# penumbra-zone/decaf377

Hardware: AMD Instinct MI355X
Metric: decaf377 var-base scalar-mults/sec + encodes/sec at 1/2/4/8 MI355X (higher is better)
Workload: dtype u32

## Files before the change

### decaf377_amd/csrc/curve.hpp

```cpp
#pragma once
#include "fq29.hpp"
#include "fqs29.hpp"

namespace d377 {

#include "constants.inc"

constexpr int GT_STRIDE = 12;
constexpr int S_HASH_BITS = 12;
struct SqrtTables {
  const uint32_t* gtab;
  const uint8_t* s_lookup;
  uint32_t* inv_fail;
};

#include "s_hash.inc"

D377_HD uint32_t s_hash_raw(const fe& x) {
  return ((x.l[0] ^ (x.l[1] << 3)) * D377_S_HASH_K) >> (32 - S_HASH_BITS);
}
D377_HD uint32_t s_hash(const fe& x) {
  D377_B(bound_require(x.vq < 1.0535, "s_lookup key must be below q + 2^248"));
  return s_hash_raw(x);
}
// ... 765 lines not shown
  F g = fe_sub(a, b);
  F f = fe_add(g, c);
  ge_of<F> r;
  r.x = fe_mul(e, f); r.y = fe_mul(g, h); r.z = fe_mul(f, g);
  r.t = p.t;
  if (with_t) r.t = fe_mul(e, h);
  return r;
}

D377_HD ge_of<fes> ge_double_neg_sq(const ge_of<fes>& p, bool with_t) {
  fes a = fe_sqr(p.x), b = fe_sqr(p.y);
  fes c = fe_sqr2x(p.z);
  fes s_ = fe_sqr(fe_sub(p.x, p.y));
  fes h = fe_add(a, b);
  fes e = fe_sub(h, s_);
  fes g = fe_sub(a, b);
  fes f = fe_add(g, c);
  ge_of<fes> r;
  r.x = fe_mul(e, f); r.y = fe_mul(g, h); r.z = fe_mul(f, g);
  r.t = p.t;
  if (with_t) r.t = fe_mul(e, h);
  return r;
}

D377_HD ge ge_double_latency(const ge& p) { return ge_double_fast(p, true); }

template <class F>
D377_HD gec_of<F> ge_to_cached(const ge_of<F>& p) {
  gec_of<F> c;
  if constexpr (std::is_same<F, fes>::value) c.ypx = fe_add(p.y, p.x);
  else c.ypx = fe_carry(fe_add(p.y, p.x));
  c.ymx = fe_sub(p.y, p.x);
  c.z2 = fe_dbl(p.z);
  c.kt = fe_mul(fe_as<F>(fe_const(FE_K)), p.t);
  return c;
}

template <class F>
D377_HD ge_of<F> ge_add_cached(const ge_of<F>& p, const gec_of<F>& q, bool neg, bool with_t) {
  F a = fe_mul(fe_sub_nc(p.y, p.x), q.ymx);
  F b = fe_mul(fe_add(p.y, p.x), q.ypx);
  F c = fe_mul(p.t, q.kt);
  F d = fe_mul(p.z, q.z2);
  F e = fe_sub(b, a), h = fe_add(b, a);
  F dmc = fe_sub(d, c), dpc = fe_add(d, c);
  F f = fe_select(neg, dpc, dmc), g = fe_select(neg, dmc, dpc);
  ge_of<F> r;
  r.x = fe_mul(e, f); r.y = fe_mul(g, h); r.z = fe_mul(f, g);
  r.t = p.t;
  if (with_t) r.t = fe_mul(e, h);
  return r;
}

struct gea { fe ypx, ymx, kt; };
D377_HD ge ge_add_affine(const ge& p, const gea& q, bool neg, bool with_t) {
  fe a = fe_mul(fe_sub_nc(p.y, p.x), q.ymx);
  fe b = fe_mul(fe_add(p.y, p.x), q.ypx);
  fe c = fe_mul(p.t, q.kt);
  fe d = fe_dbl(p.z);
  fe e = fe_sub(b, a), h = fe_add(b, a);
  fe dmc = fe_sub(d, c), dpc = fe_carry(fe_add(d, c));
  fe f = fe_select(neg, dpc, dmc), g = fe_select(neg, dmc, dpc);
  ge r;
  r.x = fe_mul(e, f); r.y = fe_mul(g, h); r.z = fe_mul(f, g);
  r.t = p.t;
  if (with_t) r.t = fe_mul(e, h);
  return r;
}

D377_HD gea gea_from_affine(const fe& x, const fe& y) {
  gea c;
  c.ypx = fe_carry(fe_add(y, x));
  c.ymx = fe_sub(y, x);
  c.kt = fe_mul(fe_mul(fe_const(FE_K), x), y);
  return c;
}
D377_HD ge ge_from_cached_affine(const gea& q, bool neg) {
  const fe one = fe_const(FE_ONE);
  ge r;
  r.x = fe_mul(fe_sub(q.ypx, fe_mul(q.ymx, one)), one);
  r.y = fe_mul(fe_add(q.ypx, q.ymx), one);
  r.z = fe_const(FE_TWO);
  const fe t = fe_mul(q.kt, fe_const(FE_2_OVER_K));
  r.t = fe_select(neg, fe_neg(t), t);
  return r;
}

template <class F>
D377_HD gec_of<F> gec_identity() {
  gec_of<F> id;
  id.ypx = fe_as<F>(fe_const(FE_ONE)); id.ymx = fe_as<F>(fe_const(FE_ONE)); id.z2 = fe_dbl(fe_as<F>(fe_const(FE_ONE)));
  id.kt = fe_as<F>(fe_zero());
  return id;
}
template <class Tab, class = void> struct tab_shares_identity { static constexpr bool value = false; };
template <class Tab> struct tab_shares_identity<Tab, std::void_t<decltype(Tab::shared_identity)>> { static constexpr bool value = Tab::shared_identity; };

template <class F = fe, class Tab>
D377_HD ge ge_scalar_mul_w4(const ge& p0, const uint32_t digits[8], Tab& tab, bool want_t = true) {
  const ge_of<F> p = ge_as<F>(p0);
  if constexpr (!tab_shares_identity<Tab>::value) tab.store(0, gec_identity<F>());
  const gec_of<F> pc = ge_to_cached(p);
  tab.store(1, pc);
  ge_of<F> acc = ge_double_fast(p, true);
  tab.store(2, ge_to_cached(acc));
#pragma unroll 1
  for (int j = 3; j <= 8; ++j) {
    acc = ge_add_cached(acc, pc, false, true);
    tab.store(j, ge_to_cached(acc));
  }
  int d = fr_digit(digits, 63);
  ge_of<F> r = ge_as<F>(ge_select(d != 0, p0, ge_identity()));
#pragma unroll 1
  for (int i = 62; i >= 0; --i) {
    d = fr_digit(digits, i);
    const bool neg = d < 0;
    const gec_of<F> e = tab.load(neg ? -d : d, neg);
#pragma unroll 1
    for (int j = 0; j < 4; ++j) r = ge_double_neg(r, j == 3);
    r = ge_add_cached(r, e, neg, want_t && i == 0);
  }
  return ge_unsigned(r);
}

template <class F = fes, class Tab>
D377_HD ge ge_scalar_mul_w4_lean(const ge& p0, const uint32_t digits[8], Tab& tab, bool want_t = true) {
  static_assert(std::is_same<F, fes>::value, "ge_double_neg_sq is priced and bounded for signed limbs");
  const ge_of<F> p = ge_as<F>(p0);
  if constexpr (!tab_shares_identity<Tab>::value) tab.store(0, gec_identity<F>());
  const gec_of<F> pc = ge_to_cached(p);
  tab.store(1, pc);
  ge_of<F> acc = ge_double_fast(p, true);
  tab.store(2, ge_to_cached(acc));
#pragma unroll 1
  for (int j = 3; j <= 8; ++j) {
    acc = ge_add_cached(acc, pc, false, true);
    tab.store(j, ge_to_cached(acc));
  }
  D377_B(bound_require(fr_digit(digits, 63) == 0 && fr_digit(digits, 62) >= 0 && fr_digit(digits, 62) <= 5,
                       "lean window chain: the scalar is not below r"));
  const int top = fr_digit(digits, 62) & 7;
  const gec_of<F> s = tab.load(top, false);
  ge_of<F> r;
  r.x = fe_carry(fe_sub(s.ypx, s.ymx)); r.y = fe_carry(fe_add(s.ypx, s.ymx)); r.z = fe_carry(s.z2);
  r.t = fe_as<F>(fe_zero());
#pragma unroll 1
  for (int i = 61; i >= 0; --i) {
    const int d = fr_digit(digits, i);
    const bool neg = d < 0;
    const gec_of<F> e = tab.load(neg ? -d : d, neg);
#pragma unroll 1
    for (int j = 0; j < 4; ++j) r = ge_double_neg_sq(r, j == 3);
    r = ge_add_cached(r, e, neg, want_t && i == 0);
  }
  return ge_unsigned(r);
}

D377_HD void fr_recode_signed256(const uint32_t k[8], int digits[32]) {
  uint32_t carry = 0;
#pragma unroll
  for (int i = 0; i < 32; ++i) {
    uint32_t d = ((k[i >> 2] >> (8 * (i & 3))) & 255u) + carry;
    carry = (d >= 128u) ? 1u : 0u;
    digits[i] = (int)d - (int)(carry << 8);
  }
}

#ifndef D377_FB_BITS
#define D377_FB_BITS 23
#endif
constexpr unsigned long long FB_R_TOP = 0x4aad95ull;
template <int BITS>
struct FbShape {
  static constexpr int bits = BITS;
  static constexpr int windows = (252 + BITS - 1) / BITS;
  static constexpr int entries = (1 << (BITS - 1)) + 1;
  static constexpr int top_bit = BITS * (windows - 1);
  static_assert(BITS >= 4 && BITS <= 23 && top_bit >= 228 && BITS * windows >= 252, "comb width");
  static_assert((FB_R_TOP >> (top_bit - 228)) + 1 < (1ull << (BITS - 1)), "the top digit of a scalar below r must not carry out");
  static_assert(windows >= 2, "the first window is peeled off the loop");
};
constexpr int FB_BITS = D377_FB_BITS;
constexpr int FB_WINDOWS = FbShape<FB_BITS>::windows;
constexpr int FB_ENTRIES = FbShape<FB_BITS>::entries;
template <int BITS = FB_BITS>
D377_HD int fb_digit(const uint32_t k[8], int i, uint32_t& carry) {
  const int bit = BITS * i, wi = bit >> 5, sh = bit & 31;
  uint32_t v = k[wi] >> sh;
  if (sh + BITS > 32 && wi + 1 < 8) v |= k[wi + 1] << (32 - sh);
  const uint32_t dd = (v & ((1u << BITS) - 1u)) + carry;
  carry = (dd >= (1u << (BITS - 1))) ? 1u : 0u;
  return (int)dd - (int)(carry << BITS);
}
template <int BITS = FB_BITS, class FTab>
D377_HD ge ge_scalar_mul_base_w8(const uint32_t k[8], const FTab& ftab, bool want_t = true) {
  constexpr int W = FbShape<BITS>::windows;
  uint32_t carry = 0;
  int d = fb_digit<BITS>(k, 0, carry);
  bool neg = d < 0;
  gea e = ftab.load(0, neg ? -d : d, neg);
  ge r;
  {
    const gea cur = e;
    const bool neg_cur = neg;
    d = fb_digit<BITS>(k, 1, carry);
    neg = d < 0;
    e = ftab.load(1, neg ? -d : d, neg);
    r = ge_from_cached_affine(cur, neg_cur);
  }
#pragma unroll 1
  for (int i = 1; i < W; ++i) {
    const gea cur = e;
    const bool neg_cur = neg;
    if (i + 1 < W) {
      d = fb_digit<BITS>(k, i + 1, carry);
      neg = d < 0;
      e = ftab.load(i + 1, neg ? -d : d, neg);
    }
    r = ge_add_affine(r, cur, neg_cur, want_t || i + 1 < W);
  }
  return r;
}
template <int BITS, class FTab, class KLoad>
D377_HD ge ge_fixed_msm_w8(int m, KLoad&& kload, const FTab& ftab, bool want_t = true) {
  constexpr int W = FbShape<BITS>::windows;
  uint32_t k[8];
  kload(0, k);
  uint32_t carry = 0;
  int d = fb_digit<BITS>(k, 0, carry);
  bool neg = d < 0;
  gea e = ftab.load(0, 0, neg ? -d : d, neg);
  ge r;
  {
    const gea cur = e;
    const bool neg_cur = neg;
    d = fb_digit<BITS>(k, 1, carry);
    neg = d < 0;
    e = ftab.load(0, 1, neg ? -d : d, neg);
    r = ge_from_cached_affine(cur, neg_cur);
  }
  const int total = m * W;
  int j = 0, i = 1;
#pragma unroll 1
  for (int s = 1; s < total; ++s) {
    const gea cur = e;
    const bool neg_cur = neg;
    if (s + 1 < total) {
      if (++i == W) {
        i = 0;
        ++j;
        kload(j, k);
        carry = 0;
      }
      d = fb_digit<BITS>(k, i, carry);
      neg = d < 0;
      e = ftab.load(j, i, neg ? -d : d, neg);
    }
    r = ge_add_affine(r, cur, neg_cur, want_t || s + 1 < total);
  }
  return r;
}
template <class FTab>
struct FbIndexedTabs {
  const FTab& tabs;
  int comb;
  D377_HD gea load(int, int i, int c, bool swap) const { return tabs.load(comb, i, c, swap); }
};
template <int BITS, class FTab, class TLoad>
D377_HD ge ge_fixed_msm_indexed_w8(int t, TLoad&& tload, const FTab& ftab, bool want_t = true) {
  FbIndexedTabs<FTab> it{ftab, 0};
  return ge_fixed_msm_w8<BITS>(t, [&](int j, uint32_t k[8]) { it.comb = tload(j, k); }, it, want_t);
}

D377_HD fe fe_pow_words(const fe& x, const uint32_t (&e)[8]) {
  fe r = fe_const(FE_ONE);
#pragma unroll 1
  for (int i = 255; i >= 0; --i) {
    r = fe_sqr(r);
    if ((e[i >> 5] >> (i & 31)) & 1u) r = fe_mul(r, x);
  }
  return r;
}
D377_HD fe fe_invert_pow(const fe& x) {
  const uint32_t ee[8] = {0xFFFFFFFFu, FQ_MODULUS_W_LIT[1] - 1u, FQ_MODULUS_W_LIT[2], FQ_MODULUS_W_LIT[3],
                          FQ_MODULUS_W_LIT[4], FQ_MODULUS_W_LIT[5], FQ_MODULUS_W_LIT[6], FQ_MODULUS_W_LIT[7]};
  return fe_pow_words(x, ee);
}

template <class PT>
D377_HD fe fe_invert_chain(const fe& x, PT& pt) {
  return fe_mul(fe_sqr_n(fe_pow_m12(x, pt), 48), fe_pow_2_47_m1(x));
}

D377_HD void fr_half_words(uint32_t k[8]) {
  const uint32_t odd = k[0] & 1u;
  uint64_t c = 0;
#pragma unroll
  for (int i = 0; i < 8; ++i) { c += (uint64_t)k[i] + (odd ? FR_ORDER_W_LIT[i] : 0u); k[i] = (uint32_t)c; c >>= 32; }
#pragma unroll
  for (int i = 0; i < 8; ++i) k[i] = (k[i] >> 1) | (i < 7 ? (k[i + 1] << 31) : 0u);
}

#ifndef D377_DCB_K
#define D377_DCB_K 8
#endif
constexpr int DCB_K = D377_DCB_K;
// ... 153 lines not shown
```

### decaf377_amd/csrc/d377.hip

```cpp
#include <hip/hip_runtime.h>
#include <stdint.h>
#include <stdio.h>
#include <stdlib.h>
#include <string.h>
#include <chrono>
#include <mutex>
#include <new>
#include <thread>
#include <type_traits>
#include <vector>

#include "../../include/decaf377_amd.h"
#include "curve.hpp"
#include "device_util.hpp"
#include "dcb.hpp"
#include "quad_ops.hpp"
#include "row_ops.hpp"
#include "host_state.hpp"
#include "codec_chunked.hpp"
#include "fixed_comb.hpp"

using namespace d377;

thread_local char d377_g_err[512] = "";

namespace {

template <class F>
struct GlobalTab {
  static_assert(std::is_same<F, fes>::value, "the packed slots hold signed-limb elements");
  static constexpr bool shared_identity = true;
  uint32_t* base;
  const uint32_t* ident;
  size_t nthreads, tid;
  __device__ __forceinline__ void store(int j, const gec_of<F>& c) {
    uint32_t* p = base + ((size_t)j * nthreads + tid) * VB_ENTRY_WORDS;
    slot_pack_store(p, c.ypx); slot_pack_store(p + PACKED_SLOT, c.ymx);
    slot_pack_store(p + 2 * PACKED_SLOT, c.z2); slot_pack_store(p + 3 * PACKED_SLOT, c.kt);
  }
  __device__ __forceinline__ gec_of<F> load(int j, bool swap) const {
    const uint32_t* own = base + ((size_t)j * nthreads + tid) * VB_ENTRY_WORDS;
    const uint32_t* p = j == 0 ? ident : own;
    gec_of<F> c;
    c.ypx = slot_unpack_load<F>(p + (swap ? PACKED_SLOT : 0));
    c.ymx = slot_unpack_load<F>(p + (swap ? 0 : PACKED_SLOT));
    c.z2 = slot_unpack_load<F>(p + 2 * PACKED_SLOT);
    c.kt = slot_unpack_load<F>(p + 3 * PACKED_SLOT);
    return c;
  }
};
template <int BITS>
struct FixedTab {
  const uint32_t* base;
  __device__ __forceinline__ gea load(int i, int j, bool swap) const {
    return pt_load_affine(base + ((size_t)i * FbShape<BITS>::entries + j) * FBW_ENTRY_WORDS, swap);
  }
};

__device__ fe fe_pow_u32(const fe& x, uint32_t e) {
  int top = 31 - __clz((int)e);
  fe r = x;
#pragma unroll 1
  for (int i = top - 1; i >= 0; --i) {
    r = fe_sqr(r);
    if ((e >> i) & 1u) r = fe_mul(r, x);
  }
  return r;
}

__global__ void __launch_bounds__(BLOCK) k_init_gtab(uint32_t* gtab) {
  const int idx = blockIdx.x * BLOCK + threadIdx.x;
  if (idx >= 6 * 256) return;
  const int t = idx >> 8, nu = idx & 255;
  fe base = fe_sqr_n(fe_const(FE_SQRT_G), 8 * t);
  fe v = nu == 0 ? fe_const(FE_ONE) : fe_pow_u32(base, (uint32_t)nu);
  v = fe_mul_strict(v, fe_const(FE_ONE));
  uint32_t* p = gtab + (size_t)idx * GT_STRIDE;
#pragma unroll
  for (int i = 0; i < NL; ++i) p[i] = v.l[i];
  p[9] = 0; p[10] = 0; p[11] = 0;
}

__global__ void k_init_vb_identity(uint32_t* rec) {
  if (blockIdx.x != 0 || threadIdx.x != 0) return;
  const gec_of<fes> id = gec_identity<fes>();
  slot_pack_store(rec, id.ypx); slot_pack_store(rec + PACKED_SLOT, id.ymx);
  slot_pack_store(rec + 2 * PACKED_SLOT, id.z2); slot_pack_store(rec + 3 * PACKED_SLOT, id.kt);
}

__global__ void __launch_bounds__(BLOCK) k_init_slookup(uint8_t* s_lookup, uint32_t* keys ,
                                                        int* collisions) {
  const int nu = threadIdx.x;
  fe b39 = fe_sqr_n(fe_const(FE_SQRT_G_INV), 39);
  fe v = nu == 0 ? fe_const(FE_ONE) : fe_pow_u32(b39, (uint32_t)nu);
  fe c = fe_reduce_once(fe_mul_strict(v, fe_const(FE_ONE)));
  keys[2 * nu] = s_hash_raw(c);
  uint32_t h2 = 0xFFFFFFFFu;
  if (c.l[NL - 1] < (1u << 16)) {
    fe cq = fe_add(c, fe_const(Q_LIMBS));
    uint32_t carry = 0;
    fe n;
#pragma unroll
    for (int i = 0; i < NL; ++i) {
      uint32_t t = cq.l[i] + carry;
      if (i < NL - 1) { n.l[i] = t & MASK29; carry = t >> RB; } else n.l[i] = t;
    }
    h2 = s_hash_raw(n);
  }
  keys[2 * nu + 1] = h2;
  for (int i = threadIdx.x; i < (1 << S_HASH_BITS); i += BLOCK) s_lookup[i] = 0;
  __syncthreads();
  if (threadIdx.x == 0) {
    int coll = 0;
    for (int k = 0; k < 256; ++k)
      for (int r = 0; r < 2; ++r) {
        uint32_t h = keys[2 * k + r];
        if (h == 0xFFFFFFFFu) continue;
        for (int k2 = 0; k2 < k; ++k2)
          for (int r2 = 0; r2 < 2; ++r2)
            if (keys[2 * k2 + r2] == h) ++coll;
        s_lookup[h] = (uint8_t)k;
      }
    *collisions = coll;
  }
}

template <int FB_BITS>
__global__ void k_init_fbase_bases(uint32_t* bases) {
  constexpr int FB_WINDOWS = FbShape<FB_BITS>::windows;
  if (blockIdx.x != 0 || threadIdx.x != 0) return;
  ge p = ge_generator();
#pragma unroll 1
  for (int i = 0; i < FB_WINDOWS; ++i) {
    slot_store(bases + (size_t)i * 4 * SLOT, p.x); slot_store(bases + (size_t)i * 4 * SLOT + SLOT, p.y);
    slot_store(bases + (size_t)i * 4 * SLOT + 2 * SLOT, p.z); slot_store(bases + (size_t)i * 4 * SLOT + 3 * SLOT, p.t);
#pragma unroll 1
    for (int k = 0; k < FB_BITS; ++k) p = ge_double(p);
  }
}
__global__ void __launch_bounds__(BLOCK, WAVES_PER_SIMD) k_sqrt_ratio_zeta(SqrtTables T, const uint8_t* num32,
                                                           const uint8_t* den32, size_t n,
                                                           uint8_t* root32, uint8_t* was_square, int min_curve_root, DcbScratch dcb) {
  D377_POW_LDS();
  D377_DCB_BEGIN(root32);
  dcb_rounds<1, false>(n, io, pt,
    [&](size_t i, int j) {
      uint32_t wd[8];
      load32(den32, i, wd);
      dcb_put_den(io, 0, j, fe_from_words_mod_order_strict(wd));
    },
    [&](size_t i, int j, const uint32_t (*invw)[8], bool have) {
      uint32_t wn[8], wd[8], wr[8];
      load32(num32, i, wn);
      load32(den32, i, wd);
      fe inv = fe_from_words(invw[0]);
      fe r;
      const bool ws = fe_sqrt_ratio_zeta<false>(T, pt, fe_from_words_mod_order_strict(wn), fe_from_words_mod_order_strict(wd), &r,
                                                min_curve_root != 0, &inv, have);
      fe_to_bytes_words(r, wr);
      store32(root32, i, wr);
      was_square[i] = ws ? 1 : 0;
    });
  D377_DCB_END();
}

constexpr int CODEC_CHUNKED_MIN = 2;
__global__ void __launch_bounds__(BLOCK, WAVES_PER_SIMD) k_decompress(SqrtTables T, const uint8_t* enc32, size_t n,
                                                      uint64_t* xyzt, uint8_t* status) {
  D377_POW_LDS();
  for (size_t i = (size_t)blockIdx.x * BLOCK + threadIdx.x; i < n; i += (size_t)gridDim.x * BLOCK) {
    uint32_t w[8];
    load32(enc32, i, w);
    ge g;
    const uint32_t bad = ge_decompress(T, pt, w, &g);
    status[i] = (uint8_t)bad;
    if (bad) {
      uint8_t* b = reinterpret_cast<uint8_t*>(xyzt);
      store32_zero(b, 4 * i); store32_zero(b, 4 * i + 1); store32_zero(b, 4 * i + 2); store32_zero(b, 4 * i + 3);
    } else {
      store_ge_mont256(xyzt, i, g);
    }
  }
}

__global__ void __launch_bounds__(BLOCK, WAVES_PER_SIMD) k_decompress_chunked(SqrtTables T, const uint8_t* enc32, size_t n,
                                                              uint64_t* xyzt, uint8_t* status, DcbScratch dcb) {
  D377_POW_LDS();
  D377_DCB_BEGIN(xyzt);
  dcb_rounds<1, false, false>(n, io, pt,
    [&](size_t i, int j) {
      uint32_t w[8];
      load32(enc32, i, w);
      dcb_put_den(io, 0, j, ge_decompress_den(w));
    },
    [&](size_t i, int, const uint32_t (*invw)[8], bool) {
      uint32_t w[8];
      load32(enc32, i, w);
      const fe inv = fe_from_words(invw[0]);
      ge g;
      const uint32_t bad = ge_decompress(T, pt, w, &g, &inv);
      status[i] = (uint8_t)bad;
      if (bad) {
        uint8_t* b = reinterpret_cast<uint8_t*>(xyzt);
        store32_zero(b, 4 * i); store32_zero(b, 4 * i + 1); store32_zero(b, 4 * i + 2); store32_zero(b, 4 * i + 3);
      } else {
        store_ge_mont256(xyzt, i, g);
      }
    });
  D377_DCB_END();
}

__global__ void __launch_bounds__(BLOCK, WAVES_PER_SIMD) k_compress(SqrtTables T, const uint64_t* xyzt, size_t n,
                                                    uint8_t* enc32) {
  D377_POW_LDS();
  for (size_t i = (size_t)blockIdx.x * BLOCK + threadIdx.x; i < n; i += (size_t)gridDim.x * BLOCK) {
    uint32_t w[8];
    ge_compress(T, pt, load_ge_mont256(xyzt, i), w);
    store32(enc32, i, w);
  }
}

__global__ void __launch_bounds__(BLOCK, WAVES_PER_SIMD) k_roundtrip(SqrtTables T, const uint8_t* enc32, size_t n,
                                                     uint8_t* out32, uint8_t* status) {
  D377_POW_LDS();
  for (size_t i = (size_t)blockIdx.x * BLOCK + threadIdx.x; i < n; i += (size_t)gridDim.x * BLOCK) {
    uint32_t w[8];
    load32(enc32, i, w);
    ge g;
    const uint32_t bad = ge_decompress(T, pt, w, &g);
    ge_compress(T, pt, g, w, bad == 0);
    status[i] = (uint8_t)bad;
    if (bad) store32_zero(out32, i); else store32(out32, i, w);
  }
}

__global__ void __launch_bounds__(BLOCK, WAVES_PER_SIMD) k_encode_to_curve(SqrtTables T, const uint8_t* fq32, size_t n,
                                                           uint8_t* out32, DcbScratch dcb) {
  D377_POW_LDS();
  D377_DCB_BEGIN(out32);
  dcb_rounds<1, true>(n, io, pt,
    [&](size_t i, int j) {
      uint32_t w[8];
      load32(fq32, i, w);
      dcb_put_den(io, 0, j, ge_elligator_den(fe_from_words_mod_order(w)));
    },
    [&](size_t i, int j, const uint32_t (*invw)[8], bool have) {
      uint32_t w[8];
      load32(fq32, i, w);
      fe inv = fe_from_words(invw[0]);
      fe s, t;
      ge_elligator_st(T, pt, fe_from_words_mod_order(w), &s, &t, &inv, have);
      D377_INVARIANT(T, ge_from_jacobi_st(s, t), true);
      dcb_put(io, j, ge_dcb_from_jacobi_st(s, t));
    });
  D377_DCB_END();
}

struct Words8 { uint32_t w[8]; };
template <class PT>
__device__ __forceinline__ Words8 hash_exceptional_words(SqrtTables T, PT pt, Words8 a1, Words8 a2) {
  fe s1, t1, s2, t2, unused = fe_zero();
  ge_elligator_st(T, pt, fe_from_words_mod_order(a1.w), &s1, &t1, &unused, false);
  ge_elligator_st(T, pt, fe_from_words_mod_order(a2.w), &s2, &t2, &unused, false);
  Words8 r;
  ge_compress(T, pt, ge_add(ge_from_jacobi_st(s1, t1), ge_from_jacobi_st(s2, t2)), r.w);
  return r;
}
template <class PT>
__device__ __forceinline__ void hash_exceptional_pair(SqrtTables T, PT pt, const uint8_t* r1, const uint8_t* r2, size_t i, uint32_t w[8]) {
  Words8 a1, a2;
  load32(r1, i, a1.w);
  load32(r2, i, a2.w);
  const Words8 r = hash_exceptional_words(T, pt, a1, a2);
#pragma unroll
  for (int k = 0; k < 8; ++k) w[k] = r.w[k];
}
__global__ void __launch_bounds__(BLOCK, WAVES_PER_SIMD) k_hash_to_curve(SqrtTables T, const uint8_t* r1, const uint8_t* r2,
                                                         size_t n, uint8_t* out32, DcbScratch dcb) {
  D377_POW_LDS();
  D377_DCB_BEGIN(out32);
  uint32_t flagged = 0;
  dcb_rounds<2, true>(n, io, pt,
    [&](size_t i, int j) {
      uint32_t w[8];
      load32(r1, i, w);
      dcb_put_den(io, 0, j, ge_elligator_den(fe_from_words_mod_order(w)));
      load32(r2, i, w);
      dcb_put_den(io, 1, j, ge_elligator_den(fe_from_words_mod_order(w)));
    },
    [&](size_t i, int j, const uint32_t (*invw)[8], bool have) {
      uint32_t w[8];
      load32(r1, i, w);
      fe inv = fe_from_words(invw[0]);
      fe s1, t1, s2, t2;
      ge_elligator_st(T, pt, fe_from_words_mod_order(w), &s1, &t1, &inv, have);
      load32(r2, i, w);
      inv = fe_from_words(invw[1]);
      ge_elligator_st(T, pt, fe_from_words_mod_order(w), &s2, &t2, &inv, have);
      D377_INVARIANT(T, ge_from_jacobi_st(s1, t1), true);
      D377_INVARIANT(T, ge_from_jacobi_st(s2, t2), true);
      bool exceptional;
      dcb_state st = ge_dcb_from_jacobi_sum(s1, t1, s2, t2, &exceptional);
#if defined(D377_CHECK_INVARIANTS)
      exceptional |= (i & 3) == 3;
#endif
      const dcb_state ne = dcb_neutral();
      st.p = fe_select(exceptional, ne.p, st.p); st.w = fe_select(exceptional, ne.w, st.w);
      st.n0 = fe_select(exceptional, ne.n0, st.n0); st.n1 = fe_select(exceptional, ne.n1, st.n1);
      dcb_put(io, j, st);
      if (exceptional) {
        flagged |= 1u << j;
        load32(r1, i, w);
        io.put(2, j, w);
        load32(r2, i, w);
        io.put(3, j, w);
      }
    },
    [&](DcbIO& io2, int cnt) {
      if (__any(flagged != 0)) {
#pragma unroll 1
        for (int j = 0; j < cnt; ++j) {
          const bool mine = ((flagged >> j) & 1u) != 0;
          if (!__any(mine)) continue;
          Words8 a1, a2;
          io2.get(2, j, a1.w);
          io2.get(3, j, a2.w);
          const Words8 r = hash_exceptional_words(T, pt, a1, a2);
          if (mine) io2.emit(j, r.w);
        }
      }
      flagged = 0;
    });
  D377_DCB_END();
}

__global__ void __launch_bounds__(BLOCK, WAVES_PER_SIMD) k_scalar_mul_var(SqrtTables T, const uint8_t* enc32,
                                                          const uint8_t* scalar32, size_t n, uint8_t* out32,
                                                          uint8_t* status, uint32_t* scratch, const uint32_t* vb_identity,
                                                          DcbScratch dcb) {
  D377_POW_LDS();
  D377_DCB_BEGIN(out32);
  GlobalTab<fes> tab;
  tab.base = scratch;
  tab.ident = vb_identity;
  tab.nthreads = (size_t)dcb.nslots * BLOCK;
  tab.tid = io.lane;
  dcb_rounds<1, true, false>(n, io, pt,
    [&](size_t i, int j) {
      uint32_t w[8];
      load32(enc32, i, w);
      dcb_put_den(io, 0, j, ge_decompress_den(w));
    },
    [&](size_t i, int j, const uint32_t (*invw)[8], bool have) {
      uint32_t w[8], k[8], dg[8];
      load32(enc32, i, w);
      load32(scalar32, i, k);
      const fe inv = fe_from_words(invw[0]);
      ge g;
      const uint32_t bad = ge_decompress<fes>(T, pt, w, &g, &inv);
      status[i] = (uint8_t)bad;
      fr_reduce_words(k);
      fr_half_words(k);
      fr_recode_signed16(k, dg);
      const ge r = ge_scalar_mul_w4_lean<fes>(g, dg, tab, DCB_WANT_T);
      D377_INVARIANT(T, r, bad == 0);
      dcb_put(io, j, ge_dcb_from_half(r, bad != 0));
    });
  D377_DCB_END();
}

template <int BITS>
__global__ void __launch_bounds__(BLOCK, FB_SETS) k_scalar_mul_base(SqrtTables T, const uint32_t* fbase,
                                                           const uint8_t* scalar32, size_t n, uint8_t* out32, DcbScratch dcb) {
  D377_POW_LDS();
  D377_DCB_BEGIN(out32);
  FixedTab<BITS> ft{fbase};
  dcb_rounds<0, true>(n, io, pt,
    [&](size_t, int) {},
    [&](size_t i, int j, const uint32_t (*)[8], bool) {
      uint32_t k[8];
      load32(scalar32, i, k);
      fr_reduce_words(k);
      fr_half_words(k);
      const ge r = ge_scalar_mul_base_w8<BITS>(k, ft, DCB_WANT_T);
      D377_INVARIANT(T, r, true);
      dcb_put(io, j, ge_dcb_from_half(r, false));
    });
  D377_DCB_END();
}

constexpr int SMALL_THREADS = 64;
constexpr int SMALL_QUADS = SMALL_THREADS / 4;
static_assert(GQ_TAB_ENTRIES == VB_ENTRIES, "the quad chain's table is the per-lane chain's: 0 .. 8 times P");
struct OneDcbIO {
  uint32_t st[4][8], parked_[8], out[8];
  __device__ __forceinline__ void put(int s, int, const uint32_t* w) { for (int k = 0; k < 8; ++k) st[s][k] = w[k]; }
  __device__ __forceinline__ void get(int s, int, uint32_t* w) const { for (int k = 0; k < 8; ++k) w[k] = st[s][k]; }
  __device__ __forceinline__ void park(int, const uint32_t* w) { for (int k = 0; k < 8; ++k) parked_[k] = w[k]; }
  __device__ __forceinline__ void parked(int, uint32_t* w) const { for (int k = 0; k < 8; ++k) w[k] = parked_[k]; }
  __device__ __forceinline__ void emit(int, const uint32_t* w) { for (int k = 0; k < 8; ++k) out[k] = w[k]; }
};
__device__ __forceinline__ fe fe_shfl_xor(const fe& a, int mask) {
  fe r;
#pragma unroll
  for (int i = 0; i < NL; ++i) r.l[i] = (uint32_t)__shfl_xor((int)a.l[i], mask);
  return r;
}
__device__ __forceinline__ fe quads16_invert(const fe& p) {
  const fe q0 = fe_shfl_xor(p, 4), p1 = fe_mul_strict(p, q0);
  const fe q1 = fe_shfl_xor(p1, 8), p2 = fe_mul_strict(p1, q1);
  const fe q2 = fe_shfl_xor(p2, 16), p3 = fe_mul_strict(p2, q2);
  const fe q3 = fe_shfl_xor(p3, 32);
  const fe inv = row::fe_invert_wave(fe_mul_strict(p3, q3));
  return fe_mul(fe_mul(fe_mul(fe_mul(inv, q3), q2), q1), q0);
}

template <bool ELEMENT>
__global__ void __launch_bounds__(SMALL_THREADS)
k_scalar_mul_var_small(SqrtTables T, const uint8_t* enc32, const uint8_t* scalar32, size_t n, uint8_t* out32, uint8_t* status) {
  __shared__ uint32_t lds_pow_[POW_TAB * NL * SMALL_THREADS];
  __shared__ uint32_t tab[SMALL_QUADS * VB_ENTRIES * GQ_WORDS];
  struct Pow64 {
    uint32_t* col;
    __device__ __forceinline__ void put(int j, const fe& v) { for (int k = 0; k < NL; ++k) col[(j * NL + k) * SMALL_THREADS] = v.l[k]; }
    __device__ __forceinline__ fe get(int j) const { fe r; for (int k = 0; k < NL; ++k) r.l[k] = col[(j * NL + k) * SMALL_THREADS]; return r; }
  } pt;
  pt.col = lds_pow_ + threadIdx.x;
  const int role = threadIdx.x & 3, quad = threadIdx.x >> 2;
  uint32_t* qtab = tab + quad * VB_ENTRIES * GQ_WORDS;
  for (size_t base = (size_t)blockIdx.x * SMALL_QUADS; base < n; base += (size_t)gridDim.x * SMALL_QUADS) {
    const bool active = base + quad < n;
    const size_t e = active ? base + quad : n - 1;
    uint32_t w[8], k[8], dg[8];
    load32(scalar32, e, k);
    ge g;
    uint32_t bad = 0;
    fr_reduce_words(k);
    if (ELEMENT) {
      g = load_ge_mont256(reinterpret_cast<const uint64_t*>(enc32), e);
    } else {
      load32(enc32, e, w);
      bad = ge_decompress(T, pt, w, &g);
      fr_half_words(k);
    }
    fr_recode_signed16(k, dg);
    const fe v = gq_scalar_mul_w4(gq_from_ge(g, role), dg, qtab, role);
    const ge r = gq_to_ge(v);
    D377_INVARIANT(T, r, bad == 0);
    if (ELEMENT) {
      if (active && role == 0) store_ge_mont256(reinterpret_cast<uint64_t*>(out32), e, r);
    } else {
      const dcb_state st = ge_dcb_from_half(r, bad != 0);
      uint32_t wo[8];
      dcb_encode_one(st, quads16_invert(st.p), wo);
      if (active && role == 0) {
        store32(out32, e, wo);
        status[e] = (uint8_t)bad;
      }
    }
    __syncthreads();
  }
}

template <int FB_BITS>
__device__ __forceinline__ fe fb_fetch_slot(const uint32_t* fbase, int role, int i, int d) {
  const int slot = gq_add_slot(role, d < 0);
  const uint32_t* src = fbase + ((size_t)i * FbShape<FB_BITS>::entries + (size_t)(d < 0 ? -d : d)) * FBW_ENTRY_WORDS + NL * (slot == 0 ? 1 : (slot == 1 ? 0 : 2));
  fe x = fe_const(FE_ONE);
  if (slot < 3) {
#pragma unroll
    for (int j = 0; j < NL; ++j) x.l[j] = src[j];
  }
  return x;
}
template <bool ELEMENT, int FB_BITS>
__global__ void __launch_bounds__(SMALL_THREADS)
k_scalar_mul_base_small(const uint32_t* fbase, const uint8_t* scalar32, size_t n, uint8_t* out) {
  constexpr int FB_WINDOWS = FbShape<FB_BITS>::windows;
  const int role = threadIdx.x & 3, quad = threadIdx.x >> 2;
  const size_t e_raw = (size_t)blockIdx.x * SMALL_QUADS + quad;
  const bool active = e_raw < n;
  const size_t e = active ? e_raw : n - 1;
  uint32_t k[8];
  load32(scalar32, e, k);
  fr_reduce_words(k);
  if (!ELEMENT) fr_half_words(k);
  uint32_t carry = 0;
  int d = fb_digit<FB_BITS>(k, 0, carry);
  fe nxt = fb_fetch_slot<FB_BITS>(fbase, role, 0, d);
  fe v = gq_from_ge(ge_identity(), role);
#pragma unroll 1
  for (int i = 0; i < FB_WINDOWS; ++i) {
    const fe cur = nxt;
    const bool neg = d < 0;
    if (i + 1 < FB_WINDOWS) {
      d = fb_digit<FB_BITS>(k, i + 1, carry);
      nxt = fb_fetch_slot<FB_BITS>(fbase, role, i + 1, d);
    }
    v = gq_add_with(v, cur, role, neg);
  }
  const ge r = gq_to_ge(v);
  if (ELEMENT) {
    if (active && role == 0) store_ge_mont256(reinterpret_cast<uint64_t*>(out), e, r);
  } else {
    const dcb_state st = ge_dcb_from_half(r, false);
    uint32_t w[8];
    dcb_encode_one(st, quads16_invert(st.p), w);
    if (active && role == 0) store32(out, e, w);
  }
}

template <bool ELEMENT>
__global__ void __launch_bounds__(64)
k_scalar_mul_var_tiny(SqrtTables T, const uint8_t* enc32, const uint8_t* scalar32, size_t n, uint8_t* out32, uint8_t* status) {
  __shared__ uint32_t tab[row::RQ_TAB_ENTRIES * row::RQ_WORDS];
  __shared__ uint32_t xrec[2 * row::RQ_WORDS];
  const int t = threadIdx.x;
// ... 1873 lines not shown
```

### decaf377_amd/csrc/fqs29.hpp

```cpp
#pragma once
#include <type_traits>
#include "fq29.hpp"

namespace d377 {

struct fes {
  int32_t l[NL];
#if defined(D377_BOUNDS)
  int64_t lo[NL], hi[NL];
  double vlo, vhi;
#endif
};

constexpr uint32_t Q2L[NL] = {0x00000002u, 0x01180000u, 0x00000085u, 0x09dbfb40u, 0x16002b35u,
                              0x0d1e5c37u, 0x0ab305a2u, 0x17a68b29u, 0x002556cau};

#if defined(D377_BOUNDS)
inline void sbound_limbs_int32(const fes& a, int64_t lim, const char* what) {
  for (int i = 0; i < NL; ++i) bound_require(a.lo[i] >= -lim && a.hi[i] < lim, what);
}
inline void sbound_product(const fes& a, const fes& b, bool square, int scale) {
  sbound_limbs_int32(a, (int64_t)1 << 31, "signed product: operand limb outside int32");
  sbound_limbs_int32(b, (int64_t)1 << 31, "signed product: operand limb outside int32");
  if (square) sbound_limbs_int32(a, (int64_t)1 << 30, "signed square: doubled limb outside int32");
  const __int128 lim = (__int128)1 << 63;
  __int128 clo = 0, chi = 0;
  for (int k = 0; k < 2 * NL - 1; ++k) {
    __int128 lo = clo, hi = chi;
    __int128 slo = clo, shi = chi;
    for (int i = 0; i < NL; ++i) {
      const int j = k - i;
      if (j < 0 || j >= NL) continue;
      const __int128 c[4] = {(__int128)a.lo[i] * b.lo[j], (__int128)a.lo[i] * b.hi[j],
                             (__int128)a.hi[i] * b.lo[j], (__int128)a.hi[i] * b.hi[j]};
      __int128 pmin = c[0], pmax = c[0];
      for (int t = 1; t < 4; ++t) { if (c[t] < pmin) pmin = c[t]; if (c[t] > pmax) pmax = c[t]; }
      pmin *= scale; pmax *= scale;
      slo += pmin; shi += pmax;
      if (pmin < 0) lo += pmin;
      if (pmax > 0) hi += pmax;
      if (j >= 1 && i < NL) {
        const __int128 red = -(__int128)MASK29 * QL[j];
        slo += red; lo += red;
      }
    }
    bound_require(lo >= -lim && hi < lim, "signed product column leaves +-2^63");
    clo = slo >= 0 ? slo >> RB : -((-slo + MASK29) >> RB);
    chi = shi >= 0 ? shi >> RB : -((-shi + MASK29) >> RB);
  }
}
inline void sbound_set_product(fes& r, const fes& a, const fes& b, double scale) {
  for (int i = 0; i < NL - 1; ++i) { r.lo[i] = 0; r.hi[i] = MASK29; }
  const double p[4] = {a.vlo * b.vlo, a.vlo * b.vhi, a.vhi * b.vlo, a.vhi * b.vhi};
  double pmin = p[0], pmax = p[0];
  for (int t = 1; t < 4; ++t) { if (p[t] < pmin) pmin = p[t]; if (p[t] > pmax) pmax = p[t]; }
  r.vlo = scale * pmin / R_OVER_Q - 1.0 - 1e-6;
  r.vhi = scale * pmax / R_OVER_Q + 1e-6;
  r.lo[NL - 1] = (int64_t)__builtin_floor(r.vlo * Q_TOP) - 1;
  r.hi[NL - 1] = (int64_t)__builtin_floor(r.vhi * Q_TOP) + 1;
  bound_require(r.lo[NL - 1] >= -((int64_t)1 << 31) && r.hi[NL - 1] < ((int64_t)1 << 31), "signed product: top limb outside int32");
}
inline void sbound_linear(fes& r, const char* what) { sbound_limbs_int32(r, (int64_t)1 << 31, what); }
#endif

template <bool SCALE2, bool SQUARE>
D377_HD fes fes_mul_ref(const fes& a, const fes& b) {
  uint64_t acc = 0;
  int32_t m[NL], a2[NL], b2[NL];
  fes r;
#pragma unroll
  for (int i = 0; i < NL; ++i) { a2[i] = (int32_t)((uint32_t)a.l[i] << 1); b2[i] = SCALE2 ? a2[i] : a.l[i]; }
#pragma unroll
  for (int k = 0; k < 2 * NL - 1; ++k) {
    const int lo = k < NL ? 0 : k - (NL - 1), hi = k < NL ? k : NL - 1;
    if (SQUARE) {
#pragma unroll
      for (int i = lo; 2 * i < k; ++i) acc += (uint64_t)((int64_t)a2[i] * b2[k - i]);
      if ((k & 1) == 0) acc += (uint64_t)((int64_t)b2[k / 2] * a.l[k / 2]);
    } else {
#pragma unroll
      for (int i = lo; i <= hi; ++i) acc += (uint64_t)((int64_t)a.l[i] * b.l[k - i]);
    }
#pragma unroll
    for (int i = lo; i < (k < NL ? k : NL); ++i) acc -= (uint64_t)((int64_t)m[i] * (int64_t)QL[k - i]);
    if (k < NL) m[k] = (int32_t)((uint32_t)acc & MASK29);
    else r.l[k - NL] = (int32_t)((uint32_t)acc & MASK29);
    acc = (uint64_t)((int64_t)acc >> RB);
  }
  r.l[NL - 1] = (int32_t)(uint32_t)acc;
  return r;
}

#if defined(__HIP_DEVICE_COMPILE__)
#define D377_ASM_NQ                                                                                     \
  "s"(-(int32_t)QL[1]), "s"(-(int32_t)QL[2]), "s"(-(int32_t)QL[3]), "s"(-(int32_t)QL[4]), "s"(-(int32_t)QL[5]), \
  "s"(-(int32_t)QL[6]), "s"(-(int32_t)QL[7]), "s"(-(int32_t)QL[8])
#endif

D377_HD fes fe_mul(const fes& a, const fes& b) {
  D377_B(sbound_product(a, b, false, 1); ++op_counts().mul);
#if defined(__HIP_DEVICE_COMPILE__)
  fes r; int64_t top; int32_t m8;
  asm(D377_ASM_SMUL : D377_ASM_OUT(r, top, m8) : D377_ASM_IN(a), D377_ASM_IN(b), D377_ASM_NQ : D377_ASM_CLOBBER);
  r.l[NL - 1] = (int32_t)top;
#else
  fes r = fes_mul_ref<false, false>(a, b);
#endif
  D377_B(sbound_set_product(r, a, b, 1.0));
  return r;
}
D377_HD fes fe_sqr(const fes& a) {
  D377_B(sbound_product(a, a, true, 1); ++op_counts().sqr);
#if defined(__HIP_DEVICE_COMPILE__)
  fes r; int64_t top; int32_t m8, t[8];
  asm(D377_ASM_SSQR : D377_ASM_OUT(r, top, m8), D377_ASM_TMP8(t) : D377_ASM_IN(a), D377_ASM_NQ : D377_ASM_CLOBBER);
  r.l[NL - 1] = (int32_t)top;
#else
  fes r = fes_mul_ref<false, true>(a, a);
#endif
  D377_B(sbound_set_product(r, a, a, 1.0));
  return r;
}
D377_HD fes fe_sqr2x(const fes& a) {
  D377_B(sbound_product(a, a, true, 2); ++op_counts().sqr);
#if defined(__HIP_DEVICE_COMPILE__)
  fes r; int64_t top; int32_t m8, t[8], t8;
  asm(D377_ASM_SSQR2X : D377_ASM_OUT(r, top, m8), D377_ASM_TMP8(t), "=&v"(t8) : D377_ASM_IN(a), D377_ASM_NQ : D377_ASM_CLOBBER);
  r.l[NL - 1] = (int32_t)top;
#else
  fes r = fes_mul_ref<true, true>(a, a);
#endif
  D377_B(sbound_set_product(r, a, a, 2.0));
  return r;
}

D377_HD fes fe_add(const fes& a, const fes& b) {
  fes r;
#pragma unroll
  for (int i = 0; i < NL; ++i) r.l[i] = (int32_t)((uint32_t)a.l[i] + (uint32_t)b.l[i]);
#if defined(D377_BOUNDS)
  for (int i = 0; i < NL; ++i) { r.lo[i] = a.lo[i] + b.lo[i]; r.hi[i] = a.hi[i] + b.hi[i]; }
  r.vlo = a.vlo + b.vlo; r.vhi = a.vhi + b.vhi;
  sbound_linear(r, "signed fe_add limb leaves int32");
#endif
  return r;
}
D377_HD fes fe_sub(const fes& a, const fes& b) {
  fes r;
#pragma unroll
  for (int i = 0; i < NL; ++i) r.l[i] = (int32_t)((uint32_t)a.l[i] - (uint32_t)b.l[i]);
#if defined(D377_BOUNDS)
  for (int i = 0; i < NL; ++i) { r.lo[i] = a.lo[i] - b.hi[i]; r.hi[i] = a.hi[i] - b.lo[i]; }
  r.vlo = a.vlo - b.vhi; r.vhi = a.vhi - b.vlo;
  sbound_linear(r, "signed fe_sub limb leaves int32");
#endif
  return r;
}
D377_HD fes fe_sub_nc(const fes& a, const fes& b) { return fe_sub(a, b); }
D377_HD fes fe_neg(const fes& a) {
  fes r;
#pragma unroll
  for (int i = 0; i < NL; ++i) r.l[i] = (int32_t)(0u - (uint32_t)a.l[i]);
#if defined(D377_BOUNDS)
  for (int i = 0; i < NL; ++i) { r.lo[i] = -a.hi[i]; r.hi[i] = -a.lo[i]; }
  r.vlo = -a.vhi; r.vhi = -a.vlo;
  sbound_linear(r, "signed fe_neg limb leaves int32");
#endif
  return r;
}
D377_HD fes fe_dbl(const fes& a) { return fe_add(a, a); }

D377_HD fes fe_carry(const fes& a) {
  fes r;
  r.l[0] = (int32_t)((uint32_t)a.l[0] & MASK29);
#pragma unroll
  for (int i = 1; i < NL - 1; ++i) r.l[i] = (int32_t)((uint32_t)a.l[i] & MASK29) + (a.l[i - 1] >> RB);
  r.l[NL - 1] = a.l[NL - 1] + (a.l[NL - 2] >> RB);
#if defined(D377_BOUNDS)
  auto low = [&](int i, int64_t& lo, int64_t& hi) {
    if (a.lo[i] >= 0 && a.hi[i] <= MASK29) { lo = a.lo[i]; hi = a.hi[i]; } else { lo = 0; hi = MASK29; }
  };
  auto sh = [](int64_t v) { return v >= 0 ? v >> RB : -((-v + MASK29) >> RB); };
  low(0, r.lo[0], r.hi[0]);
  for (int i = 1; i < NL; ++i) {
    int64_t lo, hi;
    if (i < NL - 1) low(i, lo, hi); else { lo = a.lo[i]; hi = a.hi[i]; }
    r.lo[i] = lo + sh(a.lo[i - 1]); r.hi[i] = hi + sh(a.hi[i - 1]);
  }
  r.vlo = a.vlo; r.vhi = a.vhi;
  sbound_linear(r, "signed fe_carry top limb leaves int32");
#endif
  return r;
}

D377_HD fes fe_select(bool c, const fes& a, const fes& b) {
  fes r;
#pragma unroll
  for (int i = 0; i < NL; ++i) r.l[i] = c ? a.l[i] : b.l[i];
#if defined(D377_BOUNDS)
  for (int i = 0; i < NL; ++i) { r.lo[i] = a.lo[i] < b.lo[i] ? a.lo[i] : b.lo[i]; r.hi[i] = a.hi[i] > b.hi[i] ? a.hi[i] : b.hi[i]; }
  r.vlo = a.vlo < b.vlo ? a.vlo : b.vlo; r.vhi = a.vhi > b.vhi ? a.vhi : b.vhi;
#endif
  return r;
}

D377_HD fes fes_from_fe(const fe& a) {
  fes r;
#pragma unroll
  for (int i = 0; i < NL; ++i) r.l[i] = (int32_t)a.l[i];
#if defined(D377_BOUNDS)
  for (int i = 0; i < NL; ++i) {
    bound_require(a.ub[i] < (1ull << 31), "fe -> fes: limb may not fit int32");
    r.lo[i] = 0; r.hi[i] = (int64_t)a.ub[i];
  }
  r.vlo = 0; r.vhi = a.vq;
#endif
  return r;
}
template <class F>
D377_HD F fe_as(const fe& a) {
  if constexpr (std::is_same<F, fe>::value) return a;
  else return fes_from_fe(a);
}

D377_HD fe fe_unsigned(const fe& a) { return a; }
D377_HD fe fe_unsigned(const fes& a) {
  fe t;
#pragma unroll
  for (int i = 0; i < NL; ++i) t.l[i] = (uint32_t)a.l[i] + Q2L[i];
#if defined(D377_BOUNDS)
  for (int i = 0; i < NL; ++i) {
    bound_require(a.lo[i] + (int64_t)Q2L[i] >= 0, "fes -> fe: limb + 2q may be negative");
    t.ub[i] = (uint64_t)(a.hi[i] + (int64_t)Q2L[i]);
    bound_require(t.ub[i] < (1ull << 32), "fes -> fe: limb + 2q overflows 32 bits");
  }
  t.vq = a.vhi + 2.0;
#endif
  return fe_carry(t);
}

constexpr uint32_t Q4L[NL] = {0x00000004u, 0x02300000u, 0x0000010au, 0x13b7f680u, 0x0c00566au,
                              0x1a3cb86fu, 0x15660b44u, 0x0f4d1652u, 0x004aad95u};
constexpr uint32_t Q9L[NL] = {0x00000009u, 0x14ec0000u, 0x00000256u, 0x1c5deaa0u, 0x1300c26fu, 0x1b089efau, 0x0025995au, 0x0a6d723au, 0x00a80690u};
constexpr bool is_multiple_of_q(const uint32_t (&m)[NL], uint64_t k) {
  uint64_t c = 0;
  for (int i = 0; i < NL; ++i) {
    const uint64_t t = k * QL[i] + c;
    if (m[i] != (i < NL - 1 ? (t & MASK29) : t)) return false;
    c = t >> RB;
  }
  return true;
}
static_assert(is_multiple_of_q(Q4L, 4) && is_multiple_of_q(Q9L, 9), "Q4L, Q9L must be 4q and 9q in radix 2^29");
constexpr int PACKED_WORDS = 8;
constexpr int32_t PACK_BIG_TOP = 5 << 20;

D377_HD void fes_pack256(const fes& a, uint32_t w[PACKED_WORDS]) {
  uint32_t t[NL];
  int32_t c = 0;
  const bool big = a.l[NL - 1] >= PACK_BIG_TOP;
#pragma unroll
  for (int i = 0; i < NL - 1; ++i) {
    const int32_t s = (int32_t)((uint32_t)a.l[i] + (big ? 0u - Q4L[i] : Q9L[i]) + (uint32_t)c);
    t[i] = (uint32_t)s & MASK29;
    c = s >> RB;
  }
  t[NL - 1] = (uint32_t)a.l[NL - 1] + (big ? 0u - Q4L[NL - 1] : Q9L[NL - 1]) + (uint32_t)c;
#if defined(D377_BOUNDS)
  {
    auto sh = [](int64_t v) { return v >= 0 ? v >> RB : -((-v + MASK29) >> RB); };
    int64_t clo = 0, chi = 0;
    for (int i = 0; i < NL; ++i) {
      const int64_t lo = a.lo[i] - (int64_t)Q4L[i] + clo, hi = a.hi[i] + (int64_t)Q9L[i] + chi;
      bound_require(lo >= -((int64_t)1 << 31) && hi < ((int64_t)1 << 31), "fes pack: digit sum leaves int32");
      if (i < NL - 1) bound_require(a.lo[i] > -((int64_t)1 << 30) && a.hi[i] < ((int64_t)1 << 30), "fes pack: a low limb may reach 2^30: the top limb no longer tells the value");
      clo = sh(lo); chi = sh(hi);
    }
    bound_require(a.vlo + 9.0 >= 0.0, "fes pack: value + 9q may be negative");
    bound_require(a.vhi - 4.0 < R_OVER_Q / 32.0, "fes pack: value - 4q may reach 2^256");
    bound_require(t[NL - 1] < (1u << 24), "fes pack: top digit outside [0, 2^24)");
  }
#endif
#pragma unroll
  for (int j = 0; j < PACKED_WORDS; ++j) w[j] = (t[j] >> (3 * j)) | (t[j + 1] << (RB - 3 * j));
}
D377_HD fes fes_unpack256(const uint32_t w[PACKED_WORDS]) {
  fes r;
  r.l[0] = (int32_t)(w[0] & MASK29);
#pragma unroll
  for (int i = 1; i < NL - 1; ++i) r.l[i] = (int32_t)(((w[i - 1] >> (32 - 3 * i)) | (w[i] << (3 * i))) & MASK29);
  r.l[NL - 1] = (int32_t)(w[PACKED_WORDS - 1] >> 8);
#if defined(D377_BOUNDS)
  for (int i = 0; i < NL - 1; ++i) { r.lo[i] = 0; r.hi[i] = MASK29; }
  r.lo[NL - 1] = 0; r.hi[NL - 1] = (1 << 24) - 1;
  r.vlo = 0.0; r.vhi = R_OVER_Q / 32.0;
#endif
  return r;
}

}
```

Before: 74.78 million.

## Trim variable-base window chain with Z=1 precompute and small-constant kt

Adds a specialised w4 scalar-multiplication chain for points with Z=1. Table building uses cheaper doubling and addition formulas that skip Z multiplications, and computes kt through a short-constant multiply by 2d instead of a full field multiply. The main loop walks the packed nibbles directly instead of calling fr_digit, applies the digit sign with a per-limb multiply instead of a select, and skips the T output except on the final step. The per-lane table now uses a precomputed byte stride to reduce address arithmetic. The risk is that correctness depends on the decompressed point having Z equal to one and on the new bound reasoning holding.

```diff
diff --git a/decaf377_amd/csrc/curve.hpp b/decaf377_amd/csrc/curve.hpp
--- a/decaf377_amd/csrc/curve.hpp
+++ b/decaf377_amd/csrc/curve.hpp
@@ -941,6 +941,97 @@
 #pragma unroll 1
     for (int j = 0; j < 4; ++j) r = ge_double_neg_sq(r, j == 3);
     r = ge_add_cached(r, e, neg, want_t && i == 0);
+  }
+  return ge_unsigned(r);
+}
+
+constexpr uint32_t CURVE_2D = 6042;
+D377_HD gec_of<fes> ge_to_cached_short(const ge_of<fes>& p) {
+  gec_of<fes> c;
+  c.ypx = fe_add(p.y, p.x);
+  c.ymx = fe_sub(p.y, p.x);
+  c.z2 = fe_dbl(p.z);
+  c.kt = fes_mul_small<CURVE_2D>(p.t);
+  return c;
+}
+D377_HD ge_of<fes> ge_double_fast_z1(const ge_of<fes>& p) {
+  fes a = fe_sqr(p.x), b = fe_sqr(p.y);
+  fes c = fe_as<fes>(fe_const(FE_TWO));
+  fes s_ = fe_sqr(fe_add(p.x, p.y));
+  fes h = fe_add(a, b);
+  fes e = fe_sub(h, s_);
+  fes g = fe_sub(a, b);
+  fes f = fe_add(g, c);
+  ge_of<fes> r;
+  r.x = fe_mul(e, f); r.y = fe_mul(g, h); r.z = fe_mul(f, g); r.t = fe_mul(e, h);
+  return r;
+}
+D377_HD ge_of<fes> ge_add_cached_z1(const ge_of<fes>& p, const gec_of<fes>& q) {
+  fes a = fe_mul(fe_sub(p.y, p.x), q.ymx);
+  fes b = fe_mul(fe_add(p.y, p.x), q.ypx);
+  fes c = fe_mul(p.t, q.kt);
+  fes d = fe_carry(fe_dbl(p.z));
+  fes e = fe_sub(b, a), h = fe_add(b, a);
+  fes f = fe_sub(d, c), g = fe_add(d, c);
+  ge_of<fes> r;
+  r.x = fe_mul(e, f); r.y = fe_mul(g, h); r.z = fe_mul(f, g); r.t = fe_mul(e, h);
+  return r;
+}
+D377_HD ge_of<fes> ge_add_cached_sign(const ge_of<fes>& p, const gec_of<fes>& q, int32_t sgn, bool with_t) {
+  fes a = fe_mul(fe_sub(p.y, p.x), q.ymx);
+  fes b = fe_mul(fe_add(p.y, p.x), q.ypx);
+  fes c = fes_mul_sign(fe_mul(p.t, q.kt), sgn);
+  fes d = fe_mul(p.z, q.z2);
+  fes e = fe_sub(b, a), h = fe_add(b, a);
+  fes f = fe_sub(d, c), g = fe_add(d, c);
+  ge_of<fes> r;
+  r.x = fe_mul(e, f); r.y = fe_mul(g, h); r.z = fe_mul(f, g);
+  r.t = p.t;
+  if (with_t) r.t = fe_mul(e, h);
+  return r;
+}
+template <class Tab>
+D377_HD ge ge_scalar_mul_w4_trim(const ge& p0, const uint32_t digits[8], Tab& tab, bool want_t = true) {
+#if defined(D377_BOUNDS)
+  for (int i = 0; i < NL; ++i) bound_require(p0.z.l[i] == FE_ONE[i], "trimmed window chain: the point must have Z = 1");
+#endif
+  const ge_of<fes> p = ge_as<fes>(p0);
+  if constexpr (!tab_shares_identity<Tab>::value) tab.store(0, gec_identity<fes>());
+  const gec_of<fes> pc = ge_to_cached_short(p);
+  tab.store(1, pc);
+  ge_of<fes> acc = ge_double_fast_z1(p);
+  tab.store(2, ge_to_cached_short(acc));
+#pragma unroll 1
+  for (int j = 3; j <= 8; ++j) {
+    acc = ge_add_cached_z1(acc, pc);
+    tab.store(j, ge_to_cached_short(acc));
+  }
+  D377_B(bound_require(fr_digit(digits, 63) == 0 && fr_digit(digits, 62) >= 0 && fr_digit(digits, 62) <= 5,
+                       "trimmed window chain: the scalar is not below r"));
+  const int top = fr_digit(digits, 62) & 7;
+  const gec_of<fes> s = tab.load(top, false);
+  ge_of<fes> r;
+  r.x = fe_carry(fe_sub(s.ypx, s.ymx)); r.y = fe_carry(fe_add(s.ypx, s.ymx)); r.z = fe_carry(s.z2);
+  r.t = fe_as<fes>(fe_zero());
+  uint32_t w[8];
+#pragma unroll
+  for (int k = 0; k < 8; ++k) w[k] = digits[k];
+  w[7] <<= 8;
+#pragma unroll 1
+  for (int wi = 7; wi >= 0; --wi) {
+    uint32_t cur = w[7];
+#pragma unroll
+    for (int k = 7; k >= 1; --k) w[k] = w[k - 1];
+#pragma unroll 1
+    for (int nib = wi == 7 ? 5 : 7; nib >= 0; --nib) {
+      const int d = (int32_t)cur >> 28;
+      cur <<= 4;
+      const bool neg = d < 0;
+      const gec_of<fes> e = tab.load(neg ? -d : d, neg);
+#pragma unroll 1
+      for (int j = 0; j < 4; ++j) r = ge_double_neg_sq(r, j == 3);
+      r = ge_add_cached_sign(r, e, (d >> 31) | 1, want_t && (wi | nib) == 0);
+    }
   }
   return ge_unsigned(r);
 }
diff --git a/decaf377_amd/csrc/d377.hip b/decaf377_amd/csrc/d377.hip
--- a/decaf377_amd/csrc/d377.hip
+++ b/decaf377_amd/csrc/d377.hip
@@ -46,6 +46,29 @@
     c.ymx = slot_unpack_load<F>(p + (swap ? 0 : PACKED_SLOT));
     c.z2 = slot_unpack_load<F>(p + 2 * PACKED_SLOT);
     c.kt = slot_unpack_load<F>(p + 3 * PACKED_SLOT);
+    return c;
+  }
+};
+struct GlobalTabLane {
+  static constexpr bool shared_identity = true;
+  uint32_t* own0;
+  const uint32_t* ident;
+  uint32_t stride;
+  __device__ __forceinline__ uint32_t* entry(int j) const {
+    return reinterpret_cast<uint32_t*>(reinterpret_cast<char*>(own0) + (uint64_t)(uint32_t)j * stride);
+  }
+  __device__ __forceinline__ void store(int j, const gec_of<fes>& c) {
+    uint32_t* p = entry(j);
+    slot_pack_store(p, c.ypx); slot_pack_store(p + PACKED_SLOT, c.ymx);
+    slot_pack_store(p + 2 * PACKED_SLOT, c.z2); slot_pack_store(p + 3 * PACKED_SLOT, c.kt);
+  }
+  __device__ __forceinline__ gec_of<fes> load(int j, bool swap) const {
+    const uint32_t* p = j == 0 ? ident : entry(j);
+    gec_of<fes> c;
+    c.ypx = slot_unpack_load<fes>(p + (swap ? PACKED_SLOT : 0));
+    c.ymx = slot_unpack_load<fes>(p + (swap ? 0 : PACKED_SLOT));
+    c.z2 = slot_unpack_load<fes>(p + 2 * PACKED_SLOT);
+    c.kt = slot_unpack_load<fes>(p + 3 * PACKED_SLOT);
     return c;
   }
 };
@@ -340,11 +363,10 @@
                                                           DcbScratch dcb) {
   D377_POW_LDS();
   D377_DCB_BEGIN(out32);
-  GlobalTab<fes> tab;
-  tab.base = scratch;
+  GlobalTabLane tab;
+  tab.own0 = scratch + (size_t)io.lane * VB_ENTRY_WORDS;
   tab.ident = vb_identity;
-  tab.nthreads = (size_t)dcb.nslots * BLOCK;
-  tab.tid = io.lane;
+  tab.stride = (uint32_t)dcb.nslots * BLOCK * VB_ENTRY_WORDS * 4u;
   dcb_rounds<1, true, false>(n, io, pt,
     [&](size_t i, int j) {
       uint32_t w[8];
@@ -362,7 +384,7 @@
       fr_reduce_words(k);
       fr_half_words(k);
       fr_recode_signed16(k, dg);
-      const ge r = ge_scalar_mul_w4_lean<fes>(g, dg, tab, DCB_WANT_T);
+      const ge r = ge_scalar_mul_w4_trim(g, dg, tab, DCB_WANT_T);
       D377_INVARIANT(T, r, bad == 0);
       dcb_put(io, j, ge_dcb_from_half(r, bad != 0));
     });
diff --git a/decaf377_amd/csrc/fqs29.hpp b/decaf377_amd/csrc/fqs29.hpp
--- a/decaf377_amd/csrc/fqs29.hpp
+++ b/decaf377_amd/csrc/fqs29.hpp
@@ -61,6 +61,7 @@
   bound_require(r.lo[NL - 1] >= -((int64_t)1 << 31) && r.hi[NL - 1] < ((int64_t)1 << 31), "signed product: top limb outside int32");
 }
 inline void sbound_linear(fes& r, const char* what) { sbound_limbs_int32(r, (int64_t)1 << 31, what); }
+inline unsigned long& op_counts_small() { static unsigned long c = 0; return c; }
 #endif
 
 template <bool SCALE2, bool SQUARE>
@@ -200,6 +201,66 @@
 #if defined(D377_BOUNDS)
   for (int i = 0; i < NL; ++i) { r.lo[i] = a.lo[i] < b.lo[i] ? a.lo[i] : b.lo[i]; r.hi[i] = a.hi[i] > b.hi[i] ? a.hi[i] : b.hi[i]; }
   r.vlo = a.vlo < b.vlo ? a.vlo : b.vlo; r.vhi = a.vhi > b.vhi ? a.vhi : b.vhi;
+#endif
+  return r;
+}
+
+D377_HD fes fes_mul_sign(const fes& a, int32_t s) {
+  fes r;
+#pragma unroll
+  for (int i = 0; i < NL; ++i) {
+#if defined(__HIP_DEVICE_COMPILE__)
+    asm("v_mul_lo_u32 %0, %1, %2" : "=v"(r.l[i]) : "v"(a.l[i]), "v"(s));
+#else
+    r.l[i] = (int32_t)((uint32_t)a.l[i] * (uint32_t)s);
+#endif
+  }
+#if defined(D377_BOUNDS)
+  bound_require(s == 1 || s == -1, "fes_mul_sign: the sign must be +1 or -1");
+  for (int i = 0; i < NL; ++i) {
+    r.lo[i] = a.lo[i] < -a.hi[i] ? a.lo[i] : -a.hi[i];
+    r.hi[i] = a.hi[i] > -a.lo[i] ? a.hi[i] : -a.lo[i];
+  }
+  r.vlo = a.vlo < -a.vhi ? a.vlo : -a.vhi; r.vhi = a.vhi > -a.vlo ? a.vhi : -a.vlo;
+  sbound_linear(r, "fes_mul_sign limb leaves int32");
+#endif
+  return r;
+}
+
+template <uint32_t K>
+D377_HD fes fes_mul_small(const fes& a) {
+  static_assert(K > 0 && K < (1u << 14), "a short constant");
+  constexpr int32_t C = (int32_t)(((uint64_t)K << 32) / ((uint64_t)QL[NL - 1] + 1));
+  static_assert(((uint64_t)K << 32) / ((uint64_t)QL[NL - 1] + 1) < (1ull << 31), "the reciprocal fits an int32");
+#if defined(__HIP_DEVICE_COMPILE__)
+  const int32_t m = __mulhi(a.l[NL - 1], C);
+#else
+  const int32_t m = (int32_t)(((int64_t)a.l[NL - 1] * C) >> 32);
+#endif
+  fes r;
+  int64_t carry = 0;
+#pragma unroll
+  for (int i = 0; i < NL; ++i) {
+    const int64_t acc = (int64_t)a.l[i] * (int32_t)K - (int64_t)m * (int32_t)QL[i] + carry;
+    if (i < NL - 1) { r.l[i] = (int32_t)((uint32_t)acc & MASK29); carry = acc >> RB; }
+    else r.l[i] = (int32_t)acc;
+  }
+#if defined(D377_BOUNDS)
+  {
+    sbound_limbs_int32(a, (int64_t)1 << 31, "short product: operand limb outside int32");
+    const int64_t tmax = a.hi[NL - 1] > -a.lo[NL - 1] ? a.hi[NL - 1] : -a.lo[NL - 1];
+    bound_require(tmax < ((int64_t)1 << 24), "short product: top limb outside +-2^24");
+    const double q8 = (double)QL[NL - 1];
+    const double delta = (double)tmax * ((double)K / (q8 * (q8 + 1.0)) + 1.0 / 4294967296.0) + 1e-6;
+    double low_lo = 0.0, low_hi = 0.0;
+    for (int i = 0; i < NL - 1; ++i) { low_lo = (low_lo + (double)a.lo[i]) / 536870912.0; low_hi = (low_hi + (double)a.hi[i]) / 536870912.0; }
+    for (int i = 0; i < NL - 1; ++i) { r.lo[i] = 0; r.hi[i] = MASK29; }
+    r.vlo = (double)K * (low_lo < 0 ? low_lo / q8 : low_lo / (q8 + 1.0)) - delta;
+    r.vhi = (double)K * (low_hi > 0 ? low_hi / q8 : low_hi / (q8 + 1.0)) + 1.0 + delta;
+    r.lo[NL - 1] = (int64_t)__builtin_floor(r.vlo * Q_TOP) - 1;
+    r.hi[NL - 1] = (int64_t)__builtin_floor(r.vhi * Q_TOP) + 1;
+    ++op_counts_small();
+  }
 #endif
   return r;
 }
```

Result: no change. 75.18 million, median of 6 (+0.5%).
